# AI4quantum/twisteRL

Hardware: AMD Instinct MI355X
Metric: env-steps/s (whole node) Puzzle-15 PPO rollout (higher is better)
Workload: dtype f32; 1 GPU; Puzzle-15 PPO rollout + GAE + merge: 262144 envs/GPU, difficulty 128 (<= 257 records/episode), twists {identity, transpose}, BasicPolicy 256->512->256->4|1, gamma=lambda=0.995, torch-default-init weights seed 0; total_envs=262144, parallelism=episodes sharded x1

## Files before the change

twisterl_amd/csrc/tw_api.hip:

```cpp
#include "tw_common.hpp"

#include <atomic>
#include <cmath>
#include <cstdarg>
#include <cstdio>
#include <cstdlib>
#include <cstring>
#include <map>
#include <mutex>
#include <string>
#include <utility>
#include <vector>

namespace tw {

static thread_local std::string g_err;
static thread_local hipStream_t g_stream = nullptr;

void set_error(const char *fmt, ...)
{
    char buf[1024];
    va_list ap; va_start(ap, fmt);
    vsnprintf(buf, sizeof(buf), fmt, ap);
    va_end(ap);
// ... 1307 lines not shown
    for (uint64_t i = 0; i < nc && i < 16; ++i) id |= i << (4 * i);
    out->ident = id;
    return TW_OK;
}

}

extern "C" int tw_debug_episode_order(const tw_puzzle_desc *env, uint64_t seed, uint64_t episode_offset, uint64_t n, uint64_t *boards_out, uint32_t *order_out)
{
    if (!env || !boards_out || !order_out) { set_error("tw_debug_episode_order: null argument"); return TW_ERR_INVALID; }
    if (n == 0 || n > (1ull << 24)) { set_error("tw_debug_episode_order: n = %llu out of range", (unsigned long long)n); return TW_ERR_INVALID; }
    int rc = require_device(); if (rc) return rc;
    PuzzleConsts envc; rc = make_env_consts(env, &envc, 16); if (rc) return rc;
    hipStream_t s = current_stream();
    void *buf = nullptr;
    rc = scratch_alloc(&buf, n * 12 + 256 + episode_order_scratch_bytes(n), s, "device scratch (episode order)"); if (rc) return rc;
    uint64_t *b = reinterpret_cast<uint64_t *>(buf); uint32_t *o = reinterpret_cast<uint32_t *>(b + n);
    void *scr = reinterpret_cast<uint8_t *>(buf) + align_up(n * 12, 256);
    rc = launch_init_boards(envc, seed, episode_offset, n, b, s);
    if (!rc) rc = launch_episode_order(envc, b, n, o, scr, s);
    hipError_t e = rc ? hipSuccess : hipMemcpyAsync(boards_out, b, n * 8, hipMemcpyDeviceToHost, s);
    if (!rc && e == hipSuccess) e = hipMemcpyAsync(order_out, o, n * 4, hipMemcpyDeviceToHost, s);
    if (!rc && e == hipSuccess) e = hipStreamSynchronize(s);
    (void)hipFree(buf);
    if (rc) return rc;
    TW_HIP(e);
    return TW_OK;
}

static tw_env_vtable puzzle_env_table(tw_puzzle *proto)
{
    tw_env_vtable vt{};
    vt.prototype = proto; vt.num_actions = 4; vt.n_obs = (uint32_t)proto->state.size(); vt.obs_size = vt.n_obs * vt.n_obs;
    vt.clone = [](void *e) -> void * { return tw_puzzle_clone(static_cast<tw_puzzle *>(e)); };
    vt.destroy = [](void *e) { tw_puzzle_destroy(static_cast<tw_puzzle *>(e)); };
    vt.reset = [](void *e, uint64_t seed, uint64_t episode) { (void)tw_puzzle_reset(static_cast<tw_puzzle *>(e), seed, episode); };
    vt.step = [](void *e, uint32_t a) { (void)tw_puzzle_step(static_cast<tw_puzzle *>(e), a); };
    vt.observe = [](void *e, int32_t *o) {
        const tw_puzzle *q = static_cast<const tw_puzzle *>(e);
        const int64_t n = (int64_t)q->state.size();
        for (int64_t i = 0; i < n; ++i) o[i] = (int32_t)(i * n + q->state[(size_t)i]);
    };
    vt.masks = [](void *e, uint8_t *m) { (void)tw_puzzle_masks(static_cast<tw_puzzle *>(e), m); };
    vt.reward = [](void *e) -> float { return tw_puzzle_reward(static_cast<tw_puzzle *>(e)); };
    vt.is_final = [](void *e) -> int { return tw_puzzle_is_final(static_cast<tw_puzzle *>(e)); };
    vt.success = [](void *e) -> int { return tw_puzzle_solved(static_cast<tw_puzzle *>(e)); };
    return vt;
}

static int big_board_checks(const tw_puzzle_desc *env, uint32_t precision, uint64_t *depth0)
{
    if (precision != TW_PREC_F32_EXACT) { set_error("boards above 16 cells run in f32 only"); return TW_ERR_UNSUPPORTED; }
    if ((uint64_t)env->width * env->height > 64) { set_error("Puzzle %ux%u: at most 64 cells", env->width, env->height); return TW_ERR_UNSUPPORTED; }
    *depth0 = (uint64_t)env->depth_slope * env->difficulty;
    if (*depth0 + 1 > 0xfffffffeull) { set_error("Puzzle: depth_slope*difficulty too large"); return TW_ERR_UNSUPPORTED; }
    return TW_OK;
}

static int collect_big_board(const tw_puzzle_desc *env, const tw_policy *policy, const tw_ppo_params *ppo, const tw_az_params *az, tw_collected **out)
{
    uint64_t depth0 = 0;
    int rc = big_board_checks(env, ppo ? ppo->precision : az->precision, &depth0); if (rc) return rc;
    tw_puzzle *proto = tw_puzzle_create(env->width, env->height, env->difficulty, env->depth_slope, env->max_depth);
    if (!proto) return TW_ERR_INVALID;
    tw_env_vtable vt = puzzle_env_table(proto);
    rc = ppo ? tw_ppo_collect_env(&vt, policy, ppo, (uint32_t)(depth0 + 1), out) : tw_az_collect_env(&vt, policy, az, (uint32_t)(depth0 + 1), out);
    tw_puzzle_destroy(proto);
    return rc;
}

static int ppo_collect_once(const tw_puzzle_desc *env, const tw_policy *policy, const tw_ppo_params *prm, tw_collected **out, bool *out_of_range);

extern "C" int tw_ppo_collect(const tw_puzzle_desc *env, const tw_policy *policy, const tw_ppo_params *prm,
                              tw_collected **out)
{
    bool out_of_range = false;
    int rc = ppo_collect_once(env, policy, prm, out, &out_of_range);
    if (rc != TW_OK && out_of_range) {
        static std::atomic<bool> said{false};
        if (!said.exchange(true))
            fprintf(stderr, "[twisterl_hip] precision fp16x2: a weight or an activation is outside the range of the split-f16 terms "
                            "(|weight| < 4095, |embedding| < 4095, |hidden| < 255.9): such collects run in fp32\n");
        tw_ppo_params p32 = *prm;
        p32.precision = TW_PREC_F32_EXACT;
        rc = ppo_collect_once(env, policy, &p32, out, &out_of_range);
    }
    return rc;
}

static int ppo_collect_once(const tw_puzzle_desc *env, const tw_policy *policy, const tw_ppo_params *prm, tw_collected **out, bool *out_of_range)
{
    *out_of_range = false;
    if (!env || !policy || !prm || !out) { set_error("tw_ppo_collect: null argument"); return TW_ERR_INVALID; }
    *out = nullptr;
    if (prm->num_episodes == 0) {
        set_error("Something went wrong. No data in collected data chunks to merge. ");
        return TW_ERR_EMPTY;
    }
    if (prm->precision > TW_PREC_F16X2) { set_error("tw_ppo_collect: unknown precision %u", prm->precision); return TW_ERR_INVALID; }
    int rc = require_device(); if (rc) return rc;

    const uint64_t cells = (uint64_t)env->width * env->height;
    const bool big = cells > 16;
    if (big && !(cells <= 64 && policy->dev.generic && prm->precision == TW_PREC_F32_EXACT && (uint64_t)env->depth_slope * env->difficulty <= 1022 &&
                 env->max_depth != 0 && !launch_options().force_geom))
        return collect_big_board(env, policy, prm, nullptr, out);

    RolloutArgs ra{};
    rc = make_env_consts(env, &ra.env, 64); if (rc) return rc;
    ra.pol = policy->dev;
    if (ra.pol.obs_size != ra.env.n_cells * ra.env.n_cells) {
        set_error("index out of bounds: policy obs_size %d != Puzzle obs ids %d", ra.pol.obs_size, ra.env.n_cells * ra.env.n_cells);
        return TW_ERR_INVALID;
    }
    if (ra.pol.n_actions != 4) { set_error("Puzzle has 4 actions, policy has %d", ra.pol.n_actions); return TW_ERR_INVALID; }
    if (ra.pol.generic && prm->precision != TW_PREC_F32_EXACT) { set_error("tw_ppo_collect: the f16 modes exist for the one-common-layer policy shape only"); return TW_ERR_UNSUPPORTED; }
    const uint64_t E = prm->num_episodes;
    const int t_pad = ra.env.depth0 + 1;
    ra.num_episodes = E; ra.episode_offset = prm->episode_offset; ra.seed = prm->seed;

    std::lock_guard<std::mutex> lock(g_ws_mutex);
    hipStream_t s = current_stream();

    const uint64_t R = E * (uint64_t)t_pad;
    size_t cur = 0;
    auto seg = [&](size_t bytes) { size_t o = cur; cur = align_up(cur + bytes, 256); return o; };
    ra.reserve_cus = (int)(prm->reserve_cus > 0x7fffu ? 0x7fffu : prm->reserve_cus);
    const uint64_t resident = ra.pol.generic ? rollout_generic_resident_episodes(ra.pol, ra.env.n_cells, ra.reserve_cus)
                            : prm->precision == TW_PREC_F32_EXACT ? f32_resident_episodes(E, (int)ra.pol.hidden, false, ra.reserve_cus)
                                                                  : rollout_f32_resident_episodes(ra.reserve_cus);
    const bool persist = E > resident && !launch_options().no_persist && !big;
    constexpr uint32_t ROLLOUT_DRAIN_LIVE_AUTO = 96;
    uint32_t drain_live = 0;
    if (persist && prm->precision == TW_PREC_F32_EXACT && rollout_f32_hands_over(ra.pol, resident, ra.reserve_cus)) {
        const int opt = launch_options().rollout_drain;
        drain_live = opt > 0 ? (uint32_t)opt : (opt == 0 && E >= 2 * resident ? ROLLOUT_DRAIN_LIVE_AUTO : 0u);
    }
    const size_t o_rec = seg(R * sizeof(PaddedRec)), o_len = seg(E * 4), o_start = seg(E * 8),
                 o_total = seg(32),
                 o_resume = seg(drain_live ? resident * 16 : 0),
                 o_scan = seg(scan_scratch_bytes(E)), o_init = seg(persist ? E * 16 : 0), o_queue = seg(persist ? 4 : 0),
                 o_obs16 = seg(big ? R * cells * 2 : 0), o_boards = seg(persist ? E * 8 : 0), o_ordscr = seg(persist ? episode_order_scratch_bytes(E) : 0);
    void *wsp = nullptr;
    rc = ws_reserve(cur, &wsp); if (rc) return rc;
    uint8_t *ws = reinterpret_cast<uint8_t *>(wsp);
    ra.out.rec = reinterpret_cast<PaddedRec *>(ws + o_rec);
    ra.out.ep_len = reinterpret_cast<uint32_t *>(ws + o_len); ra.out.t_pad = t_pad;
    uint64_t *ep_start_ws = reinterpret_cast<uint64_t *>(ws + o_start);
    uint64_t *total_d = reinterpret_cast<uint64_t *>(ws + o_total);

    EventSet ev; rc = ev.init(); if (rc) return rc;
    tw_collect_stats st{};
    const bool reuse_path = prm->precision == TW_PREC_F32_EXACT && !big && !ra.pol.generic;
    if (reuse_path) {
        TW_HIP(hipMemsetAsync(ws + o_total + 8, 0, 12, s));
        ra.reused = reinterpret_cast<unsigned int *>(ws + o_total + 12);
        ra.reuse_off = launch_options().rollout_reuse_off ? 1u : 0u;
    }
    if (prm->precision == TW_PREC_F16X2 && ra.pol.split_range) {
        ra.range_flag = reinterpret_cast<uint32_t *>(ws + o_total + 8);
        TW_HIP(hipMemcpyAsync(ra.range_flag, ra.pol.split_range, 4, hipMemcpyDeviceToDevice, s));
    }
    if (persist) {
        ra.init_boards = reinterpret_cast<const uint4 *>(ws + o_init);
        ra.queue = reinterpret_cast<unsigned int *>(ws + o_queue);
        const unsigned int first = (unsigned int)resident;
        TW_HIP(hipMemcpyAsync(ws + o_queue, &first, 4, hipMemcpyHostToDevice, s));
        if (drain_live) {
            ra.resume = reinterpret_cast<uint4 *>(ws + o_resume);
            ra.resume_cnt = reinterpret_cast<unsigned int *>(ws + o_total + 16);
            ra.drain_queue = reinterpret_cast<unsigned int *>(ws + o_total + 20);
            ra.drain_live = drain_live;
            const unsigned int drain_first = (unsigned int)(resident / 8);
            TW_HIP(hipMemcpyAsync(ra.drain_queue, &drain_first, 4, hipMemcpyHostToDevice, s));
        }
        const bool ordered = !(launch_options().az_variant & 64);
        rc = launch_init_boards(ra.env, ra.seed, ra.episode_offset, E, ordered ? reinterpret_cast<uint64_t *>(ws + o_boards) : nullptr, s,
                                ordered ? nullptr : reinterpret_cast<uint4 *>(ws + o_init));
        if (rc) return rc;
        if (ordered) {
            rc = launch_episode_order(ra.env, reinterpret_cast<const uint64_t *>(ws + o_boards), E, nullptr, ws + o_ordscr, s, reinterpret_cast<uint4 *>(ws + o_init));
            if (rc) return rc;
        }
    }
    TW_HIP(hipEventRecord(ev.ev[0], s));
    if (big) forget_last_launch();
    uint32_t drain_blocks = 0;
    rc = big                               ? launch_rollout_big(ra, reinterpret_cast<uint16_t *>(ws + o_obs16), s, &st.rollout_blocks, &st.rollout_threads)
         : prm->precision == TW_PREC_F16   ? launch_rollout_f16(ra, s, &st.rollout_blocks, &st.rollout_threads)
         : prm->precision == TW_PREC_F16X2 ? launch_rollout_f16x2(ra, s, &st.rollout_blocks, &st.rollout_threads)
                                           : launch_rollout_f32(ra, s, &st.rollout_blocks, &st.rollout_threads, &drain_blocks);
    if (rc) return rc;
    TW_HIP(hipEventRecord(ev.ev[1], s));
    rc = launch_scan(ra.out.ep_len, E, prm->merge_order ? 1 : 0, ep_start_ws, total_d, ws + o_scan, scan_scratch_bytes(E), s);
    if (rc) return rc;
    TW_HIP(hipEventRecord(ev.ev[2], s));
    uint64_t total_and_flag[3] = {0, 0, 0};
    TW_HIP(hipMemcpyAsync(total_and_flag, total_d, ra.drain_live ? 24 : ra.range_flag || ra.reused ? 16 : 8, hipMemcpyDeviceToHost, s));
    TW_HIP(hipStreamSynchronize(s));
    if (reuse_path) {
        std::lock_guard<std::mutex> dbg(g_dbg_mutex);
        for (int i = 0; i < 16; ++i) g_dbg_counters[i] = 0;
        g_dbg_counters[0] = total_and_flag[2] & 0xffffffffull; g_dbg_counters[1] = drain_blocks;
    }
    const uint64_t total = total_and_flag[0];
    if (total_and_flag[1] & 0xffffffffull) {
        *out_of_range = true;
        set_error("precision fp16x2: an operand outside the range of the split-f16 terms");
        return TW_ERR_UNSUPPORTED;
    }
    if (total == 0 || total > R) { set_error("collect: inconsistent record count %llu (max %llu)", (unsigned long long)total, (unsigned long long)R); return TW_ERR_HIP; }

    st.padded_bytes = cur; st.forward_evals = total;
    st.reused_evals = ra.reused ? total_and_flag[1] >> 32 : 0;
    CollectTail tail{};
    tail.is_ppo = true; tail.traj = ra.out; tail.ep_start = ep_start_ws; tail.E = E; tail.total = total;
    tail.n_cells = (uint32_t)ra.env.n_cells; tail.n_actions = 4; tail.obs_size = tail.n_cells * tail.n_cells;
    tail.cell_major = !big;
    if (big) { tail.obs16 = reinterpret_cast<const uint16_t *>(ws + o_obs16); tail.obs_width = 2; }
    tail.gamma = prm->gamma; tail.lambda = prm->lambda; tail.ev = &ev; tail.stream = s; tail.stats = st;
    return collect_tail(tail, out);
}

static int az_collect_once(const tw_puzzle_desc *env, const tw_policy *policy, const tw_az_params *prm, tw_collected **out, bool *split_watchdog);

extern "C" int tw_az_collect(const tw_puzzle_desc *env, const tw_policy *policy, const tw_az_params *prm, tw_collected **out)
{
    bool split_watchdog = false;
    forget_last_launch();
    int rc = az_collect_once(env, policy, prm, out, &split_watchdog);
    if (rc != TW_OK && split_watchdog) {
        fprintf(stderr, "[twisterl_hip] self-play: the split shape's kernels did not run side by side (a profiler that serialises kernels? a shared GPU?): "
                        "%s -- retrying on the single-kernel shapes, which this process keeps from now on\n", tw_last_error());
        mcts_deep_disable_split();
        rc = az_collect_once(env, policy, prm, out, &split_watchdog);
    }
    return rc;
}

static int az_collect_once(const tw_puzzle_desc *env, const tw_policy *policy, const tw_az_params *prm, tw_collected **out, bool *split_watchdog)
{
    *split_watchdog = false;
    if (!env || !policy || !prm || !out) { set_error("tw_az_collect: null argument"); return TW_ERR_INVALID; }
    *out = nullptr;
    if (prm->num_episodes == 0) {
        set_error("Something went wrong. No data in collected data chunks to merge. ");
        return TW_ERR_EMPTY;
    }
    if (prm->precision != TW_PREC_F32_EXACT) { set_error("tw_az_collect: precision %u not implemented", prm->precision); return TW_ERR_UNSUPPORTED; }
    int rc = require_device(); if (rc) return rc;
    const uint64_t cells = (uint64_t)env->width * env->height;
    const bool big = cells > 16;
    if (big && !(cells <= 64 && policy->dev.generic && (uint64_t)env->depth_slope * env->difficulty <= 1022 && env->max_depth != 0 &&
                 !launch_options().force_geom))
        return collect_big_board(env, policy, nullptr, prm, out);

    MctsArgs ma{};
    rc = make_env_consts(env, &ma.env, 64); if (rc) return rc;
    ma.pol = policy->dev;
    if (ma.pol.obs_size != ma.env.n_cells * ma.env.n_cells) {
        set_error("index out of bounds: policy obs_size %d != Puzzle obs ids %d", ma.pol.obs_size, ma.env.n_cells * ma.env.n_cells);
        return TW_ERR_INVALID;
    }
    if (ma.pol.n_actions != 4) { set_error("Puzzle has 4 actions, policy has %d", ma.pol.n_actions); return TW_ERR_INVALID; }
    const uint64_t E = prm->num_episodes;
    const int t_pad = ma.env.depth0 + 1;
    const uint64_t cap64 = 5ull + 4ull * prm->num_mcts_searches * (prm->max_expand_depth ? prm->max_expand_depth : 1u);
    if (cap64 > 0x7fffffffull || (uint64_t)prm->num_mcts_searches * (prm->max_expand_depth ? prm->max_expand_depth : 1u) > 0xffffffffull) {
        set_error("tw_az_collect: num_mcts_searches x max_expand_depth too large"); return TW_ERR_UNSUPPORTED;
    }
    ma.num_episodes = E; ma.episode_offset = prm->episode_offset; ma.seed = prm->seed;
    ma.num_searches = prm->num_mcts_searches; ma.max_expand_depth = prm->max_expand_depth; ma.C = prm->C;
    ma.node_cap = (uint32_t)cap64;

    std::lock_guard<std::mutex> lock(g_ws_mutex);
    hipStream_t s = current_stream();

    const uint64_t R = E * (uint64_t)t_pad;
    size_t cur = 0;
    auto seg = [&](size_t bytes) { size_t o = cur; cur = align_up(cur + bytes, 256); return o; };
    ma.reserve_cus = (int)(prm->reserve_cus > 0x7fffu ? 0x7fffu : prm->reserve_cus);
    const bool deep = !big && mcts_deep_applies(ma);
    const uint64_t resident = big ? E : deep ? mcts_deep_walkers(E, ma.reserve_cus, ma.num_searches) : f32_resident_episodes(E, (int)ma.pol.hidden, true, ma.reserve_cus);
    const bool persist = !big && (deep || (E > resident && !launch_options().no_persist && !ma.pol.generic));
    const uint64_t arenas = persist ? resident : E;
    const size_t o_rec = seg(R * sizeof(PaddedRec)), o_len = seg(E * 4), o_start = seg(E * 8),
                 o_total = seg(136), o_scan = seg(scan_scratch_bytes(E)),
                 o_arena = seg(big ? arenas * cap64 * mcts_big_node_bytes() : deep ? arenas * mcts_deep_arena_bytes(cap64) : arenas * cap64 * mcts_node_bytes()),
                 o_init = seg(persist ? E * 8 : 0), o_queue = seg(persist ? 4 : 0), o_order = seg(deep ? E * 4 : 0), o_ordscr = seg(deep ? episode_order_scratch_bytes(E) : 0),
                 o_obs16 = seg(big ? R * cells * 2 : 0);
    const uint32_t tbl_entries = deep ? mcts_deep_table_entries(ma.num_searches, ma.max_expand_depth) : 0;
    const size_t tbl_bytes = (size_t)arenas * tbl_entries * 32;
    const size_t o_tbl = seg(tbl_bytes);
    const bool split = deep && mcts_deep_split(E, ma.reserve_cus, ma.num_searches);
    const size_t o_mb = seg(split ? (size_t)arenas * 256 + 256 : 0);
    rc = check_memory_fit(cur, "tw_az_collect"); if (rc) return rc;
    void *wsp = nullptr;
    rc = ws_reserve(cur, &wsp); if (rc) return rc;
    uint8_t *ws = reinterpret_cast<uint8_t *>(wsp);
    ma.out.rec = reinterpret_cast<PaddedRec *>(ws + o_rec);
    ma.out.ep_len = reinterpret_cast<uint32_t *>(ws + o_len); ma.out.t_pad = t_pad;
    uint64_t *ep_start_ws = reinterpret_cast<uint64_t *>(ws + o_start);
    uint64_t *total_d = reinterpret_cast<uint64_t *>(ws + o_total);
    ma.eval_count = reinterpret_cast<unsigned long long *>(ws + o_total + 8);
    ma.arena = reinterpret_cast<MctsNode *>(ws + o_arena);

    EventSet ev; rc = ev.init(); if (rc) return rc;
// ... 273 lines not shown
```

twisterl_amd/csrc/tw_rollout16.hip:

```cpp
#include "tw_engine16x2.hpp"

#include <cstdio>
#include <cstdlib>

namespace tw {

TW_STAMP_ARRAY(g_stamps16, 8);

template <class Eng, int NC, bool PERSIST = false>
__global__ void __launch_bounds__(256, 1) rollout_f16_kernel(const RolloutArgs a)
{
    extern __shared__ __attribute__((aligned(16))) uint8_t lds16[];
    TW_STAMP(t_kernel0);
    Eng eng;
    eng.begin1(a.pol, lds16);

    const PuzzleConsts env = a.env;
    const int j = eng.j, hh = eng.hh;
    uint64_t   e_own  = (uint64_t)blockIdx.x * Eng::EPB + (uint64_t)(eng.wave * 64 + hh * 32 + j);
    const bool v_own  = e_own < a.num_episodes;
    uint64_t   eg_own = a.episode_offset + e_own;

    auto from_board = [&](uint64_t b) {
        PuzzleLane s; s.board = b;
        const int z = blank_cell(b);
        s.zx = z % env.width; s.zy = z / env.width; s.depth = env.depth0;
        return s;
    };
    PuzzleLane own;
    own.board = env.ident; own.zx = 0; own.zy = 0; own.depth = 0;
    if (v_own) {
        if constexpr (PERSIST) {
            const uint4 ib = a.init_boards[e_own];
            e_own = ib.z; eg_own = a.episode_offset + e_own;
            own = from_board(((uint64_t)ib.y << 32) | ib.x);
        } else puzzle_reset(own, env, a.seed, eg_own);
    }
    PuzzleLane st0, st1;
    {
        PuzzleLane oth;
        oth.board = ((uint64_t)(uint32_t)__shfl_xor((int)(uint32_t)(own.board >> 32), 32, 64) << 32) |
                    (uint64_t)(uint32_t)__shfl_xor((int)(uint32_t)own.board, 32, 64);
        oth.zx = __shfl_xor(own.zx, 32, 64); oth.zy = __shfl_xor(own.zy, 32, 64); oth.depth = __shfl_xor(own.depth, 32, 64);
        st0 = hh ? oth : own; st1 = hh ? own : oth;
    }
    const bool v_oth = __shfl_xor(v_own ? 1 : 0, 32, 64) != 0;
    bool alive0 = hh ? v_oth : v_own, alive1 = hh ? v_own : v_oth;
    int      t = 0;
    uint32_t len_own = 0;
    float    out_max = 0.0f;
    uint64_t rec_base = e_own * (uint64_t)a.out.t_pad;
    bool     more = PERSIST;

    uint32_t obs_base[4];
    obs_base_words(env.n_cells, obs_base);
    float bh[5];
#pragma unroll
    for (int i = 0; i < 5; ++i) bh[i] = a.pol.bh16[i];

    eng.begin2();
    TW_STAMP_VARS(t_prev = __builtin_readcyclecounter());
    while (__syncthreads_or((alive0 || alive1) ? 1 : 0)) {
        TW_STAMP(t_top);
        TW_STAMP_ADD(eng.st[7], t_prev, t_top);
        int perm_own = -1;
        if (eng.pol.n_perms > 0) {
            const u32x4 w = rng_draw(a.seed, eg_own, (uint32_t)t, STREAM_PERM);
            perm_own = (int)u32_below(w.x, (uint32_t)eng.pol.n_perms);
        }
        const int perm_oth = __shfl_xor(perm_own, 32, 64);
        const int perm0 = hh ? perm_oth : perm_own, perm1 = hh ? perm_own : perm_oth;
        typename Eng::OneHots oh;
        eng.onehots(st0.board, perm0, oh.a0);
        eng.onehots(st1.board, perm1, oh.a1);

        TW_STAMP_USE(oh.a0[0]); TW_STAMP_USE(oh.a1[0]);
        TW_STAMP(t_fw);
        TW_STAMP_ADD(eng.st[0], t_top, t_fw);
        f32x16 out0, out1;
        eng.forward(oh, out0, out1);
        TW_STAMP(t_po);

        float lg[4];
#pragma unroll
        for (int i = 0; i < 4; ++i) lg[i] = (hh ? out1[i] : out0[i]) * Eng::OUT_SCALE + bh[i];
        const float value = (hh ? out1[4] : out0[4]) * Eng::OUT_SCALE + bh[4];
        if constexpr (Eng::SPLIT_RANGE) {
#pragma unroll
            for (int i = 0; i < 4; ++i) out_max = __builtin_elementwise_maximum(out_max, __builtin_fabsf(lg[i]));
            out_max = __builtin_elementwise_maximum(out_max, __builtin_fabsf(value));
        }
        PuzzleLane mine;
        mine.board = hh ? st1.board : st0.board; mine.zx = hh ? st1.zx : st0.zx; mine.zy = hh ? st1.zy : st0.zy;
        mine.depth = hh ? st1.depth : st0.depth;
        eng.act_perm(perm_own, lg);
        const uint32_t mb = puzzle_maskbits(mine, env);
#pragma unroll
        for (int i = 0; i < 4; ++i) lg[i] = ((mb >> i) & 1u) ? lg[i] : -1e10f;
        const float rew = puzzle_reward(mine, env);
        const u32x4 gw = rng_draw(a.seed, eg_own, (uint32_t)t, STREAM_GUMBEL);
        const int act_own = gumbel_argmax4(lg, gw);
        const bool alive_own = hh ? alive1 : alive0;
        if (alive_own) {
            uint32_t pk[4];
            obs_bytes(mine.board, obs_base, pk);
            store_rec(a.out.rec + rec_base + (uint64_t)t, pk, lg, value, rew, act_own, perm_own);
        }
        const int act_oth = __shfl_xor(act_own, 32, 64);
        const int act0 = hh ? act_oth : act_own, act1 = hh ? act_own : act_oth;
        {
            const bool fin0 = puzzle_final(st0, env), fin1 = puzzle_final(st1, env);
            PuzzleLane n0 = st0, n1 = st1;
            puzzle_step(n0, env, act0); puzzle_step(n1, env, act1);
            const bool go0 = alive0 && !fin0, go1 = alive1 && !fin1;
            st0.board = go0 ? n0.board : st0.board; st0.zx = go0 ? n0.zx : st0.zx; st0.zy = go0 ? n0.zy : st0.zy; st0.depth = go0 ? n0.depth : st0.depth;
            st1.board = go1 ? n1.board : st1.board; st1.zx = go1 ? n1.zx : st1.zx; st1.zy = go1 ? n1.zy : st1.zy; st1.depth = go1 ? n1.depth : st1.depth;
            const bool died_own = hh ? (alive1 && fin1) : (alive0 && fin0);
            len_own = died_own ? (uint32_t)t + 1u : len_own;
            alive0 = go0; alive1 = go1;
            if constexpr (PERSIST) { if (died_own) a.out.ep_len[e_own] = len_own; }
        }
        ++t;
        if constexpr (PERSIST) {
            const bool idle_own = !(hh ? alive1 : alive0);
            unsigned got = 0xffffffffu;
            if (idle_own && more) got = atomicAdd(a.queue, 1u);
            const bool took = (uint64_t)got < a.num_episodes;
            more = more && !(idle_own && !took);
            uint64_t nb = 0;
            if (took) { const uint4 ib = a.init_boards[got]; e_own = ib.z; eg_own = a.episode_offset + e_own; rec_base = e_own * (uint64_t)a.out.t_pad; t = 0; nb = ((uint64_t)ib.y << 32) | ib.x; }
            const bool took_oth = __shfl_xor(took ? 1 : 0, 32, 64) != 0;
            const uint64_t nb_oth = ((uint64_t)(uint32_t)__shfl_xor((int)(uint32_t)(nb >> 32), 32, 64) << 32) |
                                    (uint64_t)(uint32_t)__shfl_xor((int)(uint32_t)nb, 32, 64);
            const PuzzleLane n_own = from_board(nb), n_oth = from_board(nb_oth);
            const bool t0 = hh ? took_oth : took, t1 = hh ? took : took_oth;
            const PuzzleLane &n0 = hh ? n_oth : n_own, &n1 = hh ? n_own : n_oth;
            if (t0) { st0 = n0; alive0 = true; }
            if (t1) { st1 = n1; alive1 = true; }
        }
        TW_RESTAMP(t_prev);
        TW_STAMP_ADD(eng.st[6], t_po, t_prev);
    }
    TW_STAMP(t_kernel1);
    TW_STAMP_FLUSH(eng.lane == 0, g_stamps16, eng.st[0], eng.st[1], eng.st[2], t_kernel1 - t_kernel0,
                   eng.st[4], eng.st[5], eng.st[6], eng.st[7]);
    if constexpr (!PERSIST) { if (v_own) a.out.ep_len[e_own] = len_own; }
    if constexpr (Eng::SPLIT_RANGE) {
        if (!(out_max <= 3.0e38f)) atomicOr(a.range_flag, 1u);
    }
    eng.end();
}

template <class Eng, int NC, bool PERSIST>
static int launch16p(const RolloutArgs &a, hipStream_t s, uint32_t *blocks, uint32_t *threads, size_t lds_bytes)
{
    const uint64_t nb = PERSIST ? rollout_f32_resident_episodes(a.reserve_cus) / Eng::EPB : (a.num_episodes + Eng::EPB - 1) / Eng::EPB;
    if (nb == 0 || nb > 0x7fffffffull) { set_error("rollout16: bad episode count %llu", (unsigned long long)a.num_episodes); return TW_ERR_INVALID; }
    if (lds_bytes > 159 * 1024) { set_error("rollout16: %zu bytes of LDS needed, 159 KiB available", lds_bytes); return TW_ERR_UNSUPPORTED; }
    if (int rc = ensure_dynamic_lds(reinterpret_cast<const void *>(&rollout_f16_kernel<Eng, NC, PERSIST>), lds_bytes)) return rc;
    TW_STAMPS_CLEAR(g_stamps16);
    hipLaunchKernelGGL((rollout_f16_kernel<Eng, NC, PERSIST>), dim3((unsigned)nb), dim3(Eng::THREADS), lds_bytes, s, a);
    TW_HIP(hipGetLastError());
    TW_STAMPS_REPORT(g_stamps16, s, h, {
        const double nw = (double)nb * 4.0;
        fprintf(stderr, "[stamps16] per wave (cycles x100MHz ticks): pre %.0f prologue %.0f stage-body %.0f vmcnt %.0f stage-barrier %.0f heads %.0f post %.0f step-barrier %.0f\n",
                h[0] / nw, h[1] / nw, h[2] / nw, h[3] / nw, h[4] / nw, h[5] / nw, h[6] / nw, h[7] / nw);
    });
    if (blocks) *blocks = (uint32_t)nb;
    if (threads) *threads = Eng::THREADS;
    return TW_OK;
}

template <class Eng, int NC>
static int launch16(const RolloutArgs &a, hipStream_t s, uint32_t *blocks, uint32_t *threads, size_t lds_bytes)
{
    if (a.queue && a.init_boards && a.num_episodes > rollout_f32_resident_episodes(a.reserve_cus)) return launch16p<Eng, NC, true>(a, s, blocks, threads, lds_bytes);
    return launch16p<Eng, NC, false>(a, s, blocks, threads, lds_bytes);
}

template <int NHT, bool SPLIT>
static int launch16_nc(const RolloutArgs &a, hipStream_t s, uint32_t *blocks, uint32_t *threads)
{
    if constexpr (SPLIT) {
        switch (a.pol.f16_nc) {
            case 4:  return launch16<EngineS<NHT, 4>, 4>(a, s, blocks, threads, engineS_lds_bytes<NHT, 4>());
            case 9:  return launch16<EngineS<NHT, 9>, 9>(a, s, blocks, threads, engineS_lds_bytes<NHT, 9>());
            case 16: return launch16<EngineS<NHT, 16>, 16>(a, s, blocks, threads, engineS_lds_bytes<NHT, 16>());
            default: break;
        }
    } else {
        switch (a.pol.f16_nc) {
            case 4:  return launch16<Engine16<NHT, 4>, 4>(a, s, blocks, threads, engine16_lds_bytes<NHT, 4>());
            case 9:  return launch16<Engine16<NHT, 9>, 9>(a, s, blocks, threads, engine16_lds_bytes<NHT, 9>());
            case 16: return launch16<Engine16<NHT, 16>, 16>(a, s, blocks, threads, engine16_lds_bytes<NHT, 16>());
            default: break;
        }
    }
    set_error("rollout16: bad chunk count %d", a.pol.f16_nc);
    return TW_ERR_UNSUPPORTED;
}

template <bool SPLIT>
static int launch_rollout_16(const RolloutArgs &a, hipStream_t s, uint32_t *blocks, uint32_t *threads)
{
    if (a.pol.f16_nc == 0) {
        set_error("precision f16: this policy has no f16 image (needs obs ids of the form cell*n+tile with n <= 16, at most %d "
                  "twists, and twists that map cells to cells)", E16_MAXP);
        return TW_ERR_UNSUPPORTED;
    }
    if (a.env.n_cells < 1 || a.env.n_cells > 16 || a.pol.obs_size != a.env.n_cells * a.env.n_cells || a.pol.n_actions != 4 ||
        a.pol.emb % 32 != 0 || a.pol.emb < (SPLIT ? 64 : 32) || a.pol.emb > 32 * E16_MAX_KT || a.env.n_cells > a.pol.f16_nc ||
        a.out.t_pad < a.env.depth0 + 1 || (SPLIT && (!a.pol.stageS || !a.pol.t0S))) {
        set_error("rollout16: unsupported shape (n_cells=%d obs_size=%d actions=%d emb=%d hidden=%d t_pad=%d split=%d)",
                  a.env.n_cells, a.pol.obs_size, a.pol.n_actions, a.pol.emb, a.pol.hidden, a.out.t_pad, (int)SPLIT);
        return TW_ERR_UNSUPPORTED;
    }
    switch (a.pol.hidden) {
        case 32:  return launch16_nc<1, SPLIT>(a, s, blocks, threads);
        case 64:  return launch16_nc<2, SPLIT>(a, s, blocks, threads);
        case 128: return launch16_nc<4, SPLIT>(a, s, blocks, threads);
        case 256: return launch16_nc<8, SPLIT>(a, s, blocks, threads);
        default:
            set_error("rollout16: hidden size %d not in {32,64,128,256}", a.pol.hidden);
            return TW_ERR_UNSUPPORTED;
    }
}

int launch_rollout_f16(const RolloutArgs &a, hipStream_t s, uint32_t *blocks, uint32_t *threads) { return launch_rollout_16<false>(a, s, blocks, threads); }
int launch_rollout_f16x2(const RolloutArgs &a, hipStream_t s, uint32_t *blocks, uint32_t *threads) { return launch_rollout_16<true>(a, s, blocks, threads); }

}
```

Before: 604.6 million env-steps/s.

## Fast-forward f16 rollout steps by reusing cached logits for revisited states

Adds a per-episode look-back ring in LDS that records the board and twist of the last four steps. After each network forward, up to R extra steps are taken without running the MLP whenever a lane's current board and twist match those from two or four steps earlier. In that case the stored logits and value are read back from the record buffer and used again. The twist draw moves ahead one step so the key can be checked. This skips forward passes for puzzle back-and-forth moves, at the cost of extra LDS, divergence, record re-reads and some serialization inside a wave.

```diff
diff --git a/twisterl_amd/csrc/tw_api.hip b/twisterl_amd/csrc/tw_api.hip
--- a/twisterl_amd/csrc/tw_api.hip
+++ b/twisterl_amd/csrc/tw_api.hip
@@ -1483,7 +1483,7 @@
     EventSet ev; rc = ev.init(); if (rc) return rc;
     tw_collect_stats st{};
     const bool reuse_path = prm->precision == TW_PREC_F32_EXACT && !big && !ra.pol.generic;
-    if (reuse_path) {
+    if (reuse_path || (prm->precision != TW_PREC_F32_EXACT && !big && !ra.pol.generic)) {
         TW_HIP(hipMemsetAsync(ws + o_total + 8, 0, 12, s));
         ra.reused = reinterpret_cast<unsigned int *>(ws + o_total + 12);
         ra.reuse_off = launch_options().rollout_reuse_off ? 1u : 0u;
diff --git a/twisterl_amd/csrc/tw_rollout16.hip b/twisterl_amd/csrc/tw_rollout16.hip
--- a/twisterl_amd/csrc/tw_rollout16.hip
+++ b/twisterl_amd/csrc/tw_rollout16.hip
@@ -7,50 +7,176 @@
 
 TW_STAMP_ARRAY(g_stamps16, 8);
 
+#ifndef TW_REUSE16_R_F16
+#define TW_REUSE16_R_F16 2
+#endif
+#ifndef TW_REUSE16_R_SPLIT
+#define TW_REUSE16_R_SPLIT 2
+#endif
+constexpr int REUSE16_LB = 2;
+template <class Eng> constexpr int REUSE16_R = Eng::SPLIT_RANGE ? TW_REUSE16_R_SPLIT : TW_REUSE16_R_F16;
+
+constexpr int      KEY16_SLOTS = 4, KEY16_EPS = 256, KEY16_AT = 4;
+constexpr int      KEY16_TW    = KEY16_SLOTS * 2 * KEY16_EPS;
+constexpr size_t   KEY16_BYTES = (size_t)(KEY16_SLOTS * 2 + 1) * KEY16_EPS * 4;
+constexpr unsigned KEY16_EMPTY = 0xfdfdfdfdu;
+constexpr int      PERM16_UNDRAWN = -2;
+template <class Eng> constexpr size_t reuse16_lds_bytes() { return REUSE16_R<Eng> > 0 ? KEY16_AT * 4 + KEY16_BYTES : 0; }
+static_assert(KEY16_BYTES == 36 * 256 && 2 * REUSE16_LB <= KEY16_SLOTS, "look-back keys: 36 bytes per episode, the last four steps");
+static_assert(engine16_lds_bytes<8, 16>() + KEY16_AT * 4 + KEY16_BYTES <= 159 * 1024 && engineS_lds_bytes<8, 16>() + KEY16_AT * 4 + KEY16_BYTES <= 159 * 1024,
+              "the look-back keys must fit behind the largest engine image (launch16p checks every launch)");
+
+__device__ __forceinline__ void key16_clear(unsigned *keys) { keys[KEY16_TW] = KEY16_EMPTY; }
+__device__ __forceinline__ void key16_put(unsigned *keys, int t, uint64_t board, int perm)
+{
+    unsigned *e = keys + (t & (KEY16_SLOTS - 1)) * (2 * KEY16_EPS);
+    e[0] = (uint32_t)board; e[KEY16_EPS] = (uint32_t)(board >> 32);
+    reinterpret_cast<uint8_t *>(keys + KEY16_TW)[t & (KEY16_SLOTS - 1)] = (uint8_t)(perm & 0xff);
+}
+
+__device__ __forceinline__ int draw_twist16(const RolloutArgs &a, int n_perms, uint64_t eg, int t)
+{
+    const u32x4 w = rng_draw(a.seed, eg, (uint32_t)t, STREAM_PERM);
+    return (int)u32_below(w.x, (uint32_t)n_perms);
+}
+
+__device__ __forceinline__ PuzzleLane lane_from_board(uint64_t b, const PuzzleConsts &env)
+{
+    PuzzleLane s; s.board = b;
+    const int z = blank_cell(b);
+    s.zx = z % env.width; s.zy = z / env.width; s.depth = env.depth0;
+    return s;
+}
+
+struct Lane16 {
+    PuzzleLane st0, st1;
+    bool       alive0, alive1;
+    uint64_t   e_own, eg_own, rec_base;
+    int        t;
+    uint32_t   len_own;
+    bool       more;
+    int        perm_own;
+};
+
+template <bool PERSIST, bool RAW, bool ROUNDS, class Eng>
+__device__ __forceinline__ void step_tail16(const RolloutArgs &a, const PuzzleConsts &env, const Eng &eng, const uint32_t (&obs_base)[4], const float (&bh)[5],
+                                            bool on, float (&lg)[4], float value, Lane16 &s, float &out_max, unsigned *keys)
+{
+    const int hh = eng.hh;
+    if constexpr (RAW) {
+#pragma unroll
+        for (int i = 0; i < 4; ++i) lg[i] = lg[i] * Eng::OUT_SCALE + bh[i];
+        value = value * Eng::OUT_SCALE + bh[4];
+        if constexpr (Eng::SPLIT_RANGE) {
+#pragma unroll
+            for (int i = 0; i < 4; ++i) out_max = __builtin_elementwise_maximum(out_max, __builtin_fabsf(lg[i]));
+            out_max = __builtin_elementwise_maximum(out_max, __builtin_fabsf(value));
+        }
+    }
+    PuzzleLane mine;
+    mine.board = hh ? s.st1.board : s.st0.board; mine.zx = hh ? s.st1.zx : s.st0.zx; mine.zy = hh ? s.st1.zy : s.st0.zy;
+    mine.depth = hh ? s.st1.depth : s.st0.depth;
+    if constexpr (RAW) {
+        eng.act_perm(s.perm_own, lg);
+        const uint32_t mb = puzzle_maskbits(mine, env);
+#pragma unroll
+        for (int i = 0; i < 4; ++i) lg[i] = ((mb >> i) & 1u) ? lg[i] : -1e10f;
+    }
+    const float rew = puzzle_reward(mine, env);
+    const u32x4 gw = rng_draw(a.seed, s.eg_own, (uint32_t)s.t, STREAM_GUMBEL);
+    const int act_own = gumbel_argmax4(lg, gw);
+    int perm_next = s.perm_own;
+    if constexpr (ROUNDS) { if (eng.pol.n_perms > 0) perm_next = draw_twist16(a, eng.pol.n_perms, s.eg_own, s.t + 1); }
+    const bool alive_own = hh ? s.alive1 : s.alive0;
+    if (alive_own && on) {
+        uint32_t pk[4];
+        obs_bytes(mine.board, obs_base, pk);
+        store_rec(a.out.rec + s.rec_base + (uint64_t)s.t, pk, lg, value, rew, act_own, s.perm_own);
+        if constexpr (ROUNDS) key16_put(keys, s.t, mine.board, s.perm_own);
+    }
+    const int act_oth = __shfl_xor(act_own, 32, 64);
+    const int act0 = hh ? act_oth : act_own, act1 = hh ? act_own : act_oth;
+    bool on0 = true, on1 = true;
+    if constexpr (!RAW) { const bool on_oth = __shfl_xor(on ? 1 : 0, 32, 64) != 0; on0 = hh ? on_oth : on; on1 = hh ? on : on_oth; }
+    {
+        const bool fin0 = puzzle_final(s.st0, env), fin1 = puzzle_final(s.st1, env);
+        PuzzleLane n0 = s.st0, n1 = s.st1;
+        puzzle_step(n0, env, act0); puzzle_step(n1, env, act1);
+        const bool at0 = s.alive0 && on0, at1 = s.alive1 && on1;
+        const bool go0 = at0 && !fin0, go1 = at1 && !fin1;
+        s.st0.board = go0 ? n0.board : s.st0.board; s.st0.zx = go0 ? n0.zx : s.st0.zx; s.st0.zy = go0 ? n0.zy : s.st0.zy; s.st0.depth = go0 ? n0.depth : s.st0.depth;
+        s.st1.board = go1 ? n1.board : s.st1.board; s.st1.zx = go1 ? n1.zx : s.st1.zx; s.st1.zy = go1 ? n1.zy : s.st1.zy; s.st1.depth = go1 ? n1.depth : s.st1.depth;
+        const bool died_own = hh ? (at1 && fin1) : (at0 && fin0);
+        s.len_own = died_own ? (uint32_t)s.t + 1u : s.len_own;
+        if constexpr (RAW) { s.alive0 = go0; s.alive1 = go1; }
+        else { s.alive0 = s.alive0 && !(on0 && fin0); s.alive1 = s.alive1 && !(on1 && fin1); }
+        if constexpr (PERSIST) { if (died_own) a.out.ep_len[s.e_own] = s.len_own; }
+    }
+    if constexpr (RAW) ++s.t; else s.t += on ? 1 : 0;
+    if constexpr (ROUNDS) s.perm_own = on ? perm_next : s.perm_own;
+    if constexpr (PERSIST) {
+        const bool idle_own = !(hh ? s.alive1 : s.alive0);
+        unsigned got = 0xffffffffu;
+        if (idle_own && s.more) got = atomicAdd(a.queue, 1u);
+        const bool took = (uint64_t)got < a.num_episodes;
+        s.more = s.more && !(idle_own && !took);
+        uint64_t nb = 0;
+        if (took) {
+            const uint4 ib = a.init_boards[got]; s.e_own = ib.z; s.eg_own = a.episode_offset + s.e_own; s.rec_base = s.e_own * (uint64_t)a.out.t_pad; s.t = 0; nb = ((uint64_t)ib.y << 32) | ib.x;
+            if constexpr (ROUNDS) { key16_clear(keys); s.perm_own = eng.pol.n_perms > 0 ? PERM16_UNDRAWN : -1; }
+        }
+        const bool took_oth = __shfl_xor(took ? 1 : 0, 32, 64) != 0;
+        const uint64_t nb_oth = ((uint64_t)(uint32_t)__shfl_xor((int)(uint32_t)(nb >> 32), 32, 64) << 32) |
+                                (uint64_t)(uint32_t)__shfl_xor((int)(uint32_t)nb, 32, 64);
+        const PuzzleLane n_own = lane_from_board(nb, env), n_oth = lane_from_board(nb_oth, env);
+        const bool t0 = hh ? took_oth : took, t1 = hh ? took : took_oth;
+        const PuzzleLane &n0 = hh ? n_oth : n_own, &n1 = hh ? n_own : n_oth;
+        if (t0) { s.st0 = n0; s.alive0 = true; }
+        if (t1) { s.st1 = n1; s.alive1 = true; }
+    }
+}
+
 template <class Eng, int NC, bool PERSIST = false>
 __global__ void __launch_bounds__(256, 1) rollout_f16_kernel(const RolloutArgs a)
 {
     extern __shared__ __attribute__((aligned(16))) uint8_t lds16[];
+    constexpr int  R = REUSE16_R<Eng>;
+    constexpr bool ROUNDS = R > 0;
     TW_STAMP(t_kernel0);
     Eng eng;
     eng.begin1(a.pol, lds16);
 
     const PuzzleConsts env = a.env;
     const int j = eng.j, hh = eng.hh;
-    uint64_t   e_own  = (uint64_t)blockIdx.x * Eng::EPB + (uint64_t)(eng.wave * 64 + hh * 32 + j);
-    const bool v_own  = e_own < a.num_episodes;
-    uint64_t   eg_own = a.episode_offset + e_own;
-
-    auto from_board = [&](uint64_t b) {
-        PuzzleLane s; s.board = b;
-        const int z = blank_cell(b);
-        s.zx = z % env.width; s.zy = z / env.width; s.depth = env.depth0;
-        return s;
-    };
+    Lane16 s;
+    s.e_own  = (uint64_t)blockIdx.x * Eng::EPB + (uint64_t)(eng.wave * 64 + hh * 32 + j);
+    const bool v_own = s.e_own < a.num_episodes;
+    s.eg_own = a.episode_offset + s.e_own;
+
     PuzzleLane own;
     own.board = env.ident; own.zx = 0; own.zy = 0; own.depth = 0;
     if (v_own) {
         if constexpr (PERSIST) {
-            const uint4 ib = a.init_boards[e_own];
-            e_own = ib.z; eg_own = a.episode_offset + e_own;
-            own = from_board(((uint64_t)ib.y << 32) | ib.x);
-        } else puzzle_reset(own, env, a.seed, eg_own);
-    }
-    PuzzleLane st0, st1;
+            const uint4 ib = a.init_boards[s.e_own];
+            s.e_own = ib.z; s.eg_own = a.episode_offset + s.e_own;
+            own = lane_from_board(((uint64_t)ib.y << 32) | ib.x, env);
+        } else puzzle_reset(own, env, a.seed, s.eg_own);
+    }
     {
         PuzzleLane oth;
         oth.board = ((uint64_t)(uint32_t)__shfl_xor((int)(uint32_t)(own.board >> 32), 32, 64) << 32) |
                     (uint64_t)(uint32_t)__shfl_xor((int)(uint32_t)own.board, 32, 64);
         oth.zx = __shfl_xor(own.zx, 32, 64); oth.zy = __shfl_xor(own.zy, 32, 64); oth.depth = __shfl_xor(own.depth, 32, 64);
-        st0 = hh ? oth : own; st1 = hh ? own : oth;
+        s.st0 = hh ? oth : own; s.st1 = hh ? own : oth;
     }
     const bool v_oth = __shfl_xor(v_own ? 1 : 0, 32, 64) != 0;
-    bool alive0 = hh ? v_oth : v_own, alive1 = hh ? v_own : v_oth;
-    int      t = 0;
-    uint32_t len_own = 0;
-    float    out_max = 0.0f;
-    uint64_t rec_base = e_own * (uint64_t)a.out.t_pad;
-    bool     more = PERSIST;
+    s.alive0 = hh ? v_oth : v_own; s.alive1 = hh ? v_own : v_oth;
+    s.t = 0;
+    s.len_own = 0;
+    float out_max = 0.0f;
+    s.rec_base = s.e_own * (uint64_t)a.out.t_pad;
+    s.more = PERSIST;
+    s.perm_own = -1;
 
     uint32_t obs_base[4];
     obs_base_words(env.n_cells, obs_base);
@@ -58,21 +184,36 @@
 #pragma unroll
     for (int i = 0; i < 5; ++i) bh[i] = a.pol.bh16[i];
 
+    unsigned *reuse_cnt = nullptr, *keys = nullptr;
+    if constexpr (ROUNDS) {
+        reuse_cnt = reinterpret_cast<unsigned *>(lds16 + Eng::O_RING + 3 * Eng::SBYTES);
+        keys = reuse_cnt + KEY16_AT + threadIdx.x;
+        if (threadIdx.x == 0) reuse_cnt[0] = 0u;
+        key16_clear(keys);
+        if (eng.pol.n_perms > 0) s.perm_own = PERSIST ? PERM16_UNDRAWN : draw_twist16(a, eng.pol.n_perms, s.eg_own, 0);
+    }
+
     eng.begin2();
     TW_STAMP_VARS(t_prev = __builtin_readcyclecounter());
-    while (__syncthreads_or((alive0 || alive1) ? 1 : 0)) {
+    while (__syncthreads_or((s.alive0 || s.alive1) ? 1 : 0)) {
         TW_STAMP(t_top);
         TW_STAMP_ADD(eng.st[7], t_prev, t_top);
-        int perm_own = -1;
-        if (eng.pol.n_perms > 0) {
-            const u32x4 w = rng_draw(a.seed, eg_own, (uint32_t)t, STREAM_PERM);
-            perm_own = (int)u32_below(w.x, (uint32_t)eng.pol.n_perms);
-        }
-        const int perm_oth = __shfl_xor(perm_own, 32, 64);
-        const int perm0 = hh ? perm_oth : perm_own, perm1 = hh ? perm_own : perm_oth;
+        if constexpr (ROUNDS) {
+            if constexpr (PERSIST) {
+                if (__builtin_amdgcn_ballot_w64(s.perm_own == PERM16_UNDRAWN) != 0ull) {
+                    const int p = draw_twist16(a, eng.pol.n_perms, s.eg_own, s.t);
+                    s.perm_own = s.perm_own == PERM16_UNDRAWN ? p : s.perm_own;
+                }
+            }
+        } else {
+            s.perm_own = -1;
+            if (eng.pol.n_perms > 0) s.perm_own = draw_twist16(a, eng.pol.n_perms, s.eg_own, s.t);
+        }
+        const int perm_oth = __shfl_xor(s.perm_own, 32, 64);
+        const int perm0 = hh ? perm_oth : s.perm_own, perm1 = hh ? s.perm_own : perm_oth;
         typename Eng::OneHots oh;
-        eng.onehots(st0.board, perm0, oh.a0);
-        eng.onehots(st1.board, perm1, oh.a1);
+        eng.onehots(s.st0.board, perm0, oh.a0);
+        eng.onehots(s.st1.board, perm1, oh.a1);
 
         TW_STAMP_USE(oh.a0[0]); TW_STAMP_USE(oh.a1[0]);
         TW_STAMP(t_fw);
@@ -83,60 +224,41 @@
 
         float lg[4];
 #pragma unroll
-        for (int i = 0; i < 4; ++i) lg[i] = (hh ? out1[i] : out0[i]) * Eng::OUT_SCALE + bh[i];
-        const float value = (hh ? out1[4] : out0[4]) * Eng::OUT_SCALE + bh[4];
-        if constexpr (Eng::SPLIT_RANGE) {
-#pragma unroll
-            for (int i = 0; i < 4; ++i) out_max = __builtin_elementwise_maximum(out_max, __builtin_fabsf(lg[i]));
-            out_max = __builtin_elementwise_maximum(out_max, __builtin_fabsf(value));
-        }
-        PuzzleLane mine;
-        mine.board = hh ? st1.board : st0.board; mine.zx = hh ? st1.zx : st0.zx; mine.zy = hh ? st1.zy : st0.zy;
-        mine.depth = hh ? st1.depth : st0.depth;
-        eng.act_perm(perm_own, lg);
-        const uint32_t mb = puzzle_maskbits(mine, env);
-#pragma unroll
-        for (int i = 0; i < 4; ++i) lg[i] = ((mb >> i) & 1u) ? lg[i] : -1e10f;
-        const float rew = puzzle_reward(mine, env);
-        const u32x4 gw = rng_draw(a.seed, eg_own, (uint32_t)t, STREAM_GUMBEL);
-        const int act_own = gumbel_argmax4(lg, gw);
-        const bool alive_own = hh ? alive1 : alive0;
-        if (alive_own) {
-            uint32_t pk[4];
-            obs_bytes(mine.board, obs_base, pk);
-            store_rec(a.out.rec + rec_base + (uint64_t)t, pk, lg, value, rew, act_own, perm_own);
-        }
-        const int act_oth = __shfl_xor(act_own, 32, 64);
-        const int act0 = hh ? act_oth : act_own, act1 = hh ? act_own : act_oth;
-        {
-            const bool fin0 = puzzle_final(st0, env), fin1 = puzzle_final(st1, env);
-            PuzzleLane n0 = st0, n1 = st1;
-            puzzle_step(n0, env, act0); puzzle_step(n1, env, act1);
-            const bool go0 = alive0 && !fin0, go1 = alive1 && !fin1;
-            st0.board = go0 ? n0.board : st0.board; st0.zx = go0 ? n0.zx : st0.zx; st0.zy = go0 ? n0.zy : st0.zy; st0.depth = go0 ? n0.depth : st0.depth;
-            st1.board = go1 ? n1.board : st1.board; st1.zx = go1 ? n1.zx : st1.zx; st1.zy = go1 ? n1.zy : st1.zy; st1.depth = go1 ? n1.depth : st1.depth;
-            const bool died_own = hh ? (alive1 && fin1) : (alive0 && fin0);
-            len_own = died_own ? (uint32_t)t + 1u : len_own;
-            alive0 = go0; alive1 = go1;
-            if constexpr (PERSIST) { if (died_own) a.out.ep_len[e_own] = len_own; }
-        }
-        ++t;
-        if constexpr (PERSIST) {
-            const bool idle_own = !(hh ? alive1 : alive0);
-            unsigned got = 0xffffffffu;
-            if (idle_own && more) got = atomicAdd(a.queue, 1u);
-            const bool took = (uint64_t)got < a.num_episodes;
-            more = more && !(idle_own && !took);
-            uint64_t nb = 0;
-            if (took) { const uint4 ib = a.init_boards[got]; e_own = ib.z; eg_own = a.episode_offset + e_own; rec_base = e_own * (uint64_t)a.out.t_pad; t = 0; nb = ((uint64_t)ib.y << 32) | ib.x; }
-            const bool took_oth = __shfl_xor(took ? 1 : 0, 32, 64) != 0;
-            const uint64_t nb_oth = ((uint64_t)(uint32_t)__shfl_xor((int)(uint32_t)(nb >> 32), 32, 64) << 32) |
-                                    (uint64_t)(uint32_t)__shfl_xor((int)(uint32_t)nb, 32, 64);
-            const PuzzleLane n_own = from_board(nb), n_oth = from_board(nb_oth);
-            const bool t0 = hh ? took_oth : took, t1 = hh ? took : took_oth;
-            const PuzzleLane &n0 = hh ? n_oth : n_own, &n1 = hh ? n_own : n_oth;
-            if (t0) { st0 = n0; alive0 = true; }
-            if (t1) { st1 = n1; alive1 = true; }
+        for (int i = 0; i < 4; ++i) lg[i] = hh ? out1[i] : out0[i];
+        step_tail16<PERSIST, true, ROUNDS>(a, env, eng, obs_base, bh, true, lg, hh ? out1[4] : out0[4], s, out_max, keys);
+
+        if constexpr (ROUNDS) {
+            if (!a.reuse_off) {
+                bool cand = true;
+#pragma unroll 1
+                for (int r = 0; r < R; ++r) {
+                    const uint64_t board = hh ? s.st1.board : s.st0.board;
+                    const uint32_t tws = keys[KEY16_TW];
+                    bool hit = false; int back = 0;
+#pragma unroll
+                    for (int k = REUSE16_LB; k >= 1; --k) {
+                        const int sl = (s.t - 2 * k) & (KEY16_SLOTS - 1);
+                        const unsigned *e = keys + sl * (2 * KEY16_EPS);
+                        const uint32_t blo = e[0], bhi = e[KEY16_EPS];
+                        if (s.t >= 2 * k && blo == (uint32_t)board && bhi == (uint32_t)(board >> 32) &&
+                            ((tws >> (8 * sl)) & 0xffu) == (uint32_t)(s.perm_own & 0xff)) { hit = true; back = 2 * k; }
+                    }
+                    hit = hit && cand && (hh ? s.alive1 : s.alive0);
+                    if (__builtin_amdgcn_ballot_w64(hit) == 0ull) break;
+                    cand = hit;
+                    float value = 0.0f;
+#pragma unroll
+                    for (int i = 0; i < 4; ++i) lg[i] = 0.0f;
+                    if (hit) {
+                        atomicAdd(reuse_cnt, 1u);
+                        const uint4 *rec = reinterpret_cast<const uint4 *>(a.out.rec + s.rec_base + (uint64_t)(s.t - back));
+                        const uint4 q = rec[1];
+                        lg[0] = __uint_as_float(q.x); lg[1] = __uint_as_float(q.y); lg[2] = __uint_as_float(q.z); lg[3] = __uint_as_float(q.w);
+                        value = __uint_as_float(rec[2].x);
+                    }
+                    step_tail16<PERSIST, false, ROUNDS>(a, env, eng, obs_base, bh, hit, lg, value, s, out_max, keys);
+                }
+            }
         }
         TW_RESTAMP(t_prev);
         TW_STAMP_ADD(eng.st[6], t_po, t_prev);
@@ -144,7 +266,13 @@
     TW_STAMP(t_kernel1);
     TW_STAMP_FLUSH(eng.lane == 0, g_stamps16, eng.st[0], eng.st[1], eng.st[2], t_kernel1 - t_kernel0,
                    eng.st[4], eng.st[5], eng.st[6], eng.st[7]);
-    if constexpr (!PERSIST) { if (v_own) a.out.ep_len[e_own] = len_own; }
+    if constexpr (ROUNDS) {
+        if (__builtin_amdgcn_mbcnt_hi(~0u, __builtin_amdgcn_mbcnt_lo(~0u, 0u)) == 0u) {
+            const unsigned n = atomicExch(reuse_cnt, 0u);
+            if (n) atomicAdd(a.reused, n);
+        }
+    }
+    if constexpr (!PERSIST) { if (v_own) a.out.ep_len[s.e_own] = s.len_own; }
     if constexpr (Eng::SPLIT_RANGE) {
         if (!(out_max <= 3.0e38f)) atomicOr(a.range_flag, 1u);
     }
@@ -156,7 +284,9 @@
 {
     const uint64_t nb = PERSIST ? rollout_f32_resident_episodes(a.reserve_cus) / Eng::EPB : (a.num_episodes + Eng::EPB - 1) / Eng::EPB;
     if (nb == 0 || nb > 0x7fffffffull) { set_error("rollout16: bad episode count %llu", (unsigned long long)a.num_episodes); return TW_ERR_INVALID; }
+    lds_bytes += reuse16_lds_bytes<Eng>();
     if (lds_bytes > 159 * 1024) { set_error("rollout16: %zu bytes of LDS needed, 159 KiB available", lds_bytes); return TW_ERR_UNSUPPORTED; }
+    if (REUSE16_R<Eng> > 0 && !a.reused && !a.reuse_off) { set_error("rollout16: the fast-forward rounds need RolloutArgs::reused (or reuse_off)"); return TW_ERR_INVALID; }
     if (int rc = ensure_dynamic_lds(reinterpret_cast<const void *>(&rollout_f16_kernel<Eng, NC, PERSIST>), lds_bytes)) return rc;
     TW_STAMPS_CLEAR(g_stamps16);
     hipLaunchKernelGGL((rollout_f16_kernel<Eng, NC, PERSIST>), dim3((unsigned)nb), dim3(Eng::THREADS), lds_bytes, s, a);
```

After: 604.2 million env-steps/s. Within noise of the previous version (-0.1%).
